# mbitsnbites/himg

Measured on NVIDIA B200. Metric: encode+decode megapixels/sec, higher is better.
Workload: dtype int16

## Files before the change

himg_b200/csrc/api.cu:

```cuda
#include <cuda_runtime.h>

#include <algorithm>
#include <chrono>
#include <cstdlib>
#include <cstdarg>
#include <cstdio>
#include <cstring>
#include <map>
#include <mutex>
#include <string>
#include <thread>
#include <vector>

#include "../../include/himg_cuda.h"
#include "huff_dec_kernels.cuh"
#include "huff_enc_kernels.cuh"
#include "tables.h"
#include "xform_fwd3.cuh"
#include "xform_inv2.cuh"
#include "xform_avg2.cuh"
#include "xform_inv4.cuh"
#include "xform_kernels.cuh"

using namespace himgcu;

namespace {

__global__ void k_store_u32(uint32_t *__restrict__ dst, const uint32_t *__restrict__ src, int n) {
  const int i = blockIdx.x * blockDim.x + threadIdx.x;
  if (i < n) dst[i] = src[i];
}

struct DevBuf {
  void *p = nullptr;
  size_t cap = 0;
};

struct ProfRec {
  const char *name;
  cudaEvent_t a, b;
};

}

struct himgcu_ctx {
  int device = 0;
  cudaStream_t own_stream = nullptr;
  cudaStream_t stream = nullptr;
  cudaStream_t in_stream = nullptr, out_stream = nullptr;
  cudaStream_t aux_stream = nullptr;
  cudaEvent_t ev_fork = nullptr, ev_join = nullptr;
  static constexpr int kMaxLanes = 8;
  std::vector<himgcu_ctx *> lanes;
  int host_lanes = 3;
  cudaEvent_t ev_in[kMaxLanes] = {}, ev_cmp[kMaxLanes] = {}, ev_out[kMaxLanes] = {};
  std::string err;
  std::map<std::string, DevBuf> bufs;
  DevBuf full_lut;
  DevBuf signed_lut;
  void *pinned = nullptr;
  size_t pinned_cap = 0;
  void *stage[2] = {nullptr, nullptr};
  cudaEvent_t stage_ev[2] = {nullptr, nullptr};
  bool profile = false;
  std::vector<ProfRec> pending;
  std::vector<cudaEvent_t> event_pool;
  std::map<std::string, std::pair<double, int>> prof;
  std::vector<std::string> prof_names;
  uint64_t launches = 0;
  size_t max_workspace = (size_t)24 << 30;
  int item_lists = 1;
  size_t host_sub_bytes = (size_t)192 << 20;
  bool force_generic = false;
  int xform_variant = 0;
  std::string lowres_key, prefix_key;
};

namespace {

int fail(himgcu_ctx *c, int code, const char *fmt, ...) {
  char buf[512];
  va_list ap;
  va_start(ap, fmt);
  vsnprintf(buf, sizeof(buf), fmt, ap);
  va_end(ap);
  if (c) c->err = buf;
  return code;
}

#define CK(call)                                                                              \
  do {                                                                                        \
    cudaError_t e_ = (call);                                                                  \
    if (e_ != cudaSuccess)                                                                    \
      return fail(ctx, HIMGCU_ERR_CUDA, "%s failed: %s (%s:%d)", #call, cudaGetErrorString(e_), \
                  __FILE__, __LINE__);                                                        \
  } while (0)

int ensure(himgcu_ctx *ctx, const char *name, size_t bytes, void **out) {
  DevBuf &b = ctx->bufs[name];
  if (b.cap < bytes) {
    if (b.p) {
      CK(cudaStreamSynchronize(ctx->stream));
      CK(cudaFree(b.p));
      b.p = nullptr;
      b.cap = 0;
    }
    const size_t want = (bytes + 255) & ~(size_t)255;
    CK(cudaMalloc(&b.p, want));
    b.cap = want;
    ctx->lowres_key.clear();
    ctx->prefix_key.clear();
  }
  *out = b.p;
  return HIMGCU_OK;
}

#define ENSURE(name, bytes, ptr)                                             \
  do {                                                                       \
    void *p_ = nullptr;                                                      \
    int rc_ = ensure(ctx, name, (bytes), &p_);                               \
    if (rc_ != HIMGCU_OK) return rc_;                                        \
    ptr = reinterpret_cast<decltype(ptr)>(p_);                               \
  } while (0)

cudaEvent_t get_event(himgcu_ctx *ctx) {
  if (!ctx->event_pool.empty()) {
    cudaEvent_t e = ctx->event_pool.back();
    ctx->event_pool.pop_back();
    return e;
  }
  cudaEvent_t e;
  cudaEventCreate(&e);
  return e;
}

struct LaunchScope {
  himgcu_ctx *ctx;
  const char *name;
  cudaEvent_t a = nullptr, b = nullptr;
  LaunchScope(himgcu_ctx *c, const char *n) : ctx(c), name(n) {
    ++ctx->launches;
    if (ctx->profile) {
      a = get_event(ctx);
      b = get_event(ctx);
      cudaEventRecord(a, ctx->stream);
    }
  }
  ~LaunchScope() {
    if (ctx->profile) {
      cudaEventRecord(b, ctx->stream);
      ctx->pending.push_back({name, a, b});
    }
  }
};
// ... 335 lines not shown
  const int total_pairs = g.rows * (g.cols / 2);
  constexpr int TP = NCH == 1 ? kInv4ThreadsGray : kInv4ThreadsRgb;
  dim3 grid((total_pairs + TP - 1) / TP, 1, n);
  const int smem = NCH * 64 * 2 * TP + kInvTableBytes;
  CK(cudaFuncSetAttribute((k_inverse4<NCH, TP>), cudaFuncAttributeMaxDynamicSharedMemorySize, smem));
  const uint32_t pr_magic = (uint32_t)((1ull << 32) / (unsigned)(g.cols / 2)) + 1u;
  LAUNCH("k_inverse", (k_inverse4<NCH, TP>), grid, TP, smem, d_planes, d_R, g, d_inv, inv_stride, d_pixels, 1u, pr_magic);
  return HIMGCU_OK;
}

int stage_inverse(himgcu_ctx *ctx, const uint8_t *d_planes, const uint8_t *d_R, int n, const Geom &g,
                  const DecTables *d_tabs, unsigned long long tab_stride, uint8_t *d_pixels) {
  if (!ctx->force_generic && !(ctx->xform_variant & 1) && (g.h % 8) == 0 && (g.cols % 16) == 0 && (g.w % 16) == 0 &&
      (g.nch == 1 || g.nch == 3) && (reinterpret_cast<uintptr_t>(d_planes) & 15) == 0 &&
      (reinterpret_cast<uintptr_t>(d_pixels) & 15) == 0 && (reinterpret_cast<uintptr_t>(d_R) & 1) == 0) {
    if (g.nch == 1) return launch_inv4<1>(ctx, d_planes, d_R, n, g, d_tabs, tab_stride, d_pixels);
    return launch_inv4<3>(ctx, d_planes, d_R, n, g, d_tabs, tab_stride, d_pixels);
  }
  if (!ctx->force_generic && (g.w % 8) == 0 && (g.h % 8) == 0 && (g.cols % 16) == 0 &&
      (reinterpret_cast<uintptr_t>(d_planes) & 15) == 0 && (reinterpret_cast<uintptr_t>(d_pixels) & 7) == 0 &&
      (((size_t)g.w * g.nch) & 7) == 0) {
    switch (g.nch) {
      case 1: return launch_inv2<1>(ctx, d_planes, d_R, n, g, d_tabs, tab_stride, d_pixels);
      case 3: return launch_inv2<3>(ctx, d_planes, d_R, n, g, d_tabs, tab_stride, d_pixels);
      case 4: return launch_inv2<4>(ctx, d_planes, d_R, n, g, d_tabs, tab_stride, d_pixels);
      default: break;
    }
  }
  switch (g.nch) {
    case 1: return launch_inv<1>(ctx, d_planes, d_R, n, g, d_tabs, tab_stride, d_pixels);
    case 2: return launch_inv<2>(ctx, d_planes, d_R, n, g, d_tabs, tab_stride, d_pixels);
    case 3: return launch_inv<3>(ctx, d_planes, d_R, n, g, d_tabs, tab_stride, d_pixels);
    case 4: return launch_inv<4>(ctx, d_planes, d_R, n, g, d_tabs, tab_stride, d_pixels);
    default: break;
  }
  int rc = launch_inv<3>(ctx, d_planes, d_R, n, g, d_tabs, tab_stride, d_pixels, 0, g.nch);
  for (int c = 3; c < g.nch && !rc; ++c) rc = launch_inv<1>(ctx, d_planes, d_R, n, g, d_tabs, tab_stride, d_pixels, c, g.nch);
  return rc;
}

struct HuffChunkArgs {
  const uint8_t *d_in;
  HuffGeom hg;
  const char *tag;
  std::vector<uint8_t> prefix;
  int size_patch;
};

int huff_encode_items(himgcu_ctx *ctx, int n, HuffChunkArgs *chunks, int nchunks, bool riff, uint8_t *d_out,
                      size_t out_stride, uint32_t *d_sizes) {
  int *d_err;
  const bool fresh = ctx->bufs.find("enc_err") == ctx->bufs.end() || ctx->bufs["enc_err"].p == nullptr;
  ENSURE("enc_err", sizeof(int), d_err);
  if (fresh) CK(cudaMemsetAsync(d_err, 0, sizeof(int), ctx->stream));
  LayoutParams P;
  memset(&P, 0, sizeof(P));
  P.nchunks = nchunks;
  P.riff_patch = riff ? 1 : 0;
  P.out = d_out;
  P.out_stride = out_stride;
  P.sizes = d_sizes;
  P.err = d_err;
  size_t prefix_total = 0;
  for (int k = 0; k < nchunks; ++k) prefix_total += chunks[k].prefix.size();
  uint8_t *d_prefix = nullptr;
  if (prefix_total) {
    ENSURE("enc_prefix", prefix_total, d_prefix);
    std::vector<uint8_t> all;
    for (int k = 0; k < nchunks; ++k) all.insert(all.end(), chunks[k].prefix.begin(), chunks[k].prefix.end());
    const std::string key(all.begin(), all.end());
    if (ctx->prefix_key != key) {
      CK(cudaMemcpyAsync(d_prefix, all.data(), all.size(), cudaMemcpyHostToDevice, ctx->stream));
      CK(cudaStreamSynchronize(ctx->stream));
      ctx->prefix_key = key;
    }
  }
  size_t prefix_off = 0;
  TreeOut *d_trees[2];
  uint32_t *d_seghist[2], *d_bits[2], *d_pos[2];
  uint32_t *d_part[2], *d_pbits[2];
  TreeParams TP;
  memset(&TP, 0, sizeof(TP));
  ItemLists lists[2];
  for (int k = 0; k < nchunks; ++k) {
    HuffGeom &hg = chunks[k].hg;
    hg.nsub = 1;
    hg.sub_size = hg.seg_size;
    const long long ctas = (long long)n * hg.nseg, fill = hg.nseg == 1 ? 148 * 8 : 148 * 2;
    if (!ctx->force_generic && ctas < fill && hg.seg_size > 2 * kTokPiece) {
      const int want = (int)std::min<long long>(64, (fill + ctas - 1) / ctas);
      const int sub = (int)((((long long)hg.seg_size + want - 1) / want + kTokPiece - 1) / kTokPiece) * kTokPiece;
      hg.sub_size = sub;
      hg.nsub = (hg.seg_size + sub - 1) / sub;
    }
    const std::string tag = chunks[k].tag;
    ENSURE((tag + "_seghist").c_str(), (size_t)n * hg.nseg * hg.nsub * kSyms * sizeof(uint32_t), d_seghist[k]);
    ENSURE((tag + "_partstart").c_str(), (size_t)n * hg.nseg * hg.nsub * sizeof(uint32_t), d_part[k]);
    ENSURE((tag + "_trees").c_str(), (size_t)n * sizeof(TreeOut), d_trees[k]);
    ENSURE((tag + "_segbits").c_str(), (size_t)n * hg.nseg * sizeof(uint32_t), d_bits[k]);
    ENSURE((tag + "_segpos").c_str(), (size_t)n * hg.nseg * sizeof(uint32_t), d_pos[k]);
    dim3 grid(hg.nseg * hg.nsub, n);
    ItemLists &il = lists[k];
    il = ItemLists{nullptr, nullptr, nullptr, 0};
    if (!ctx->force_generic && ctx->item_lists) {
      const int ppp = (hg.sub_size + kTokPiece - 1) / kTokPiece;
      const size_t slots = (size_t)n * hg.nseg * hg.nsub * ppp;
      ENSURE((tag + "_itpos").c_str(), slots * kItemCap * sizeof(unsigned short), il.pos);
      ENSURE((tag + "_itval").c_str(), slots * kItemCap, il.val);
      ENSURE((tag + "_itcnt").c_str(), slots * sizeof(uint32_t), il.count);
      il.pieces_per_part = ppp;
    }
    ENSURE((tag + "_partbits").c_str(), (size_t)n * hg.nseg * hg.nsub * sizeof(uint32_t), d_pbits[k]);
    uint32_t *d_total = nullptr;
    if (!ctx->force_generic) {
      ENSURE((tag + "_histtotal").c_str(), (size_t)n * kSyms * sizeof(uint32_t), d_total);
      CK(cudaMemsetAsync(d_total, 0, (size_t)n * kSyms * sizeof(uint32_t), ctx->stream));
    }
    if (ctx->force_generic) LAUNCH("k_huff_hist", k_huff_hist, grid, kHuffThreads, 0, chunks[k].d_in, hg, d_seghist[k]);
    else LAUNCH("k_huff_hist", k_huff_hist2, grid, kTokThreads, 0, chunks[k].d_in, hg, d_seghist[k], il, d_total);
    TP.total[k] = d_total;
    TP.seghist[k] = d_seghist[k];
    TP.trees[k] = d_trees[k];
    TP.rows[k] = hg.nseg * hg.nsub;
    LayoutChunk &C = P.ch[k];
    C.part_bits = d_pbits[k];
    C.seghist = d_seghist[k];
    C.trees = d_trees[k];
    C.seg_bits = d_bits[k];
    C.seg_pos = d_pos[k];
    C.part_start = d_part[k];
    C.nsub = hg.nsub;
    C.prefix = chunks[k].prefix.empty() ? nullptr : d_prefix + prefix_off;
    C.prefix_len = (int)chunks[k].prefix.size();
    C.size_patch = chunks[k].size_patch;
    C.nseg = hg.nseg;
    C.framed = hg.nseg > 1 ? 1 : 0;
    prefix_off += chunks[k].prefix.size();
  }
  LAUNCH("k_huff_tree", k_huff_tree, dim3(n, nchunks), kTreeThreads, 0, TP, d_err);
  for (int k = 0; k < nchunks; ++k) {
    const int rows = chunks[k].hg.nseg * chunks[k].hg.nsub;
    LAUNCH("k_huff_layout", k_huff_segbits, dim3((rows + 7) / 8, n), 256, 0, d_seghist[k], d_trees[k], rows, d_pbits[k]);
  }
  LAUNCH("k_huff_layout", k_huff_layout, n, kLayoutThreads, 0, P);
  const size_t win_bytes = (kWinWords + 2) * sizeof(uint32_t);
  if (ctx->force_generic)
    CK(cudaFuncSetAttribute(k_huff_pack, cudaFuncAttributeMaxDynamicSharedMemorySize, (int)win_bytes));
  for (int k = 0; k < nchunks; ++k) {
    const HuffGeom &hg = chunks[k].hg;
    dim3 grid(hg.nseg * hg.nsub, n);
    if (ctx->force_generic)
      LAUNCH("k_huff_pack", k_huff_pack, grid, kHuffThreads, win_bytes, chunks[k].d_in, hg, d_trees[k], d_bits[k],
             d_pos[k], d_sizes, d_out, (unsigned long long)out_stride, d_err);
    else
      LAUNCH("k_huff_pack", k_huff_pack3, grid, kTokThreads, 0, chunks[k].d_in, hg, d_trees[k], d_bits[k], d_pos[k],
             d_part[k], d_sizes, d_out, (unsigned long long)out_stride, d_err, lists[k]);
    if (hg.nseg > 1) {
      LAUNCH("k_huff_stale", k_huff_stale, dim3((hg.nseg + 255) / 256, n), 256, 0, n, hg.nseg, d_bits[k], d_pos[k], d_sizes,
             d_out, (unsigned long long)out_stride);
    }
  }
  return HIMGCU_OK;
}

int read_err_flag(himgcu_ctx *ctx, const char *name, int *value) {
  int *d_err;
  ENSURE(name, sizeof(int), d_err);
  CK(cudaMemcpyAsync(value, d_err, sizeof(int), cudaMemcpyDeviceToHost, ctx->stream));
  CK(cudaMemsetAsync(d_err, 0, sizeof(int), ctx->stream));
  CK(cudaStreamSynchronize(ctx->stream));
  return HIMGCU_OK;
}

int enc_err_status(himgcu_ctx *ctx, int err) {
  if (err == 5) return fail(ctx, HIMGCU_ERR_UNSUPPORTED, "Huffman code longer than 32 bits");
  if (err == 99) return fail(ctx, HIMGCU_ERR_CUDA, "internal: packed size mismatch");
  if (err) return fail(ctx, HIMGCU_ERR_CAPACITY, "internal output bound exceeded");
  return HIMGCU_OK;
}

size_t per_image_encode_ws(const Geom &g) {
  return 2 * (size_t)g.nch * g.rows * g.cols + g.lres_stride + g.planes_bytes +
         (size_t)(g.rows + 1) * kSyms * 4 + 2 * sizeof(TreeOut) + (size_t)(g.rows + 1) * 8 +
         ((size_t)g.rows * ((g.seg + kTokPiece - 1) / kTokPiece) + (g.lres_size + kTokPiece - 1) / kTokPiece + 64) *
             (kItemCap * 3 + 4);
}

int encode_device(himgcu_ctx *ctx, const uint8_t *d_pixels, int n, const Geom &g, int quality, bool ycbcr,
                  uint8_t *d_out, size_t out_stride, uint32_t *d_sizes) {
  EncodeTables t;
  BuildEncodeTables(quality, ycbcr, &t);
  ContainerTemplate ct;
  BuildContainerTemplate(t, g.w, g.h, g.nch, &ct);
  uint8_t *d_L, *d_lres, *d_planes;
  ENSURE("L", (size_t)n * g.nch * g.rows * g.cols, d_L);
  ENSURE("lres", (size_t)n * g.lres_stride, d_lres);
  ENSURE("planes", (size_t)n * g.planes_bytes, d_planes);
  int rc = stage_lowres(ctx, d_pixels, n, g, ycbcr, d_L);
  if (rc) return rc;
  rc = stage_lres_encode(ctx, d_L, n, g, t, d_lres);
  if (rc) return rc;
  rc = stage_forward(ctx, d_pixels, d_L, n, g, t, d_planes);
  if (rc) return rc;
  HuffChunkArgs ch[2];
  ch[0].d_in = d_lres;
  ch[0].hg = HuffGeom{g.lres_size, g.lres_size, 1, g.lres_stride, 1, g.lres_size};
  ch[0].tag = "lres";
  ch[0].prefix = ct.head;
  ch[0].size_patch = (int)ct.head.size() - 4;
  ch[1].d_in = d_planes;
  ch[1].hg = HuffGeom{(int)g.planes_bytes, g.seg, g.rows, g.planes_bytes, 1, g.seg};
  ch[1].tag = "fres";
  ch[1].prefix = ct.mid;
  ch[1].size_patch = (int)ct.mid.size() - 4;
  return huff_encode_items(ctx, n, ch, 2, true, d_out, out_stride, d_sizes);
}

int decode_team(long long streams, int out_bytes, int base) {
  int team = base;
  while (team < kParMaxTeam && streams * team < 131072 && out_bytes / (team * 2) >= 256) team *= 2;
  return team;
}

constexpr int kDecCluster = 8;
bool use_decode_cluster(long long streams, int out_bytes) { return streams <= 16 && out_bytes >= (64 << 10); }
int launch_stream_cluster(himgcu_ctx *ctx, const char *name, int n, const uint8_t *d_in, const ChunkDesc *d_cd,
                          const DecTree *d_tree, const SegRef *d_seg, int out_seg, uint8_t *d_out,
                          unsigned long long out_stride, int *d_status, bool *launched) {
  const int threads = out_seg >= (256 << 10) ? 512 : 256;
  cudaLaunchConfig_t cfg = {};
  cfg.gridDim = dim3(kDecCluster, n);
  cfg.blockDim = dim3(threads);
  cfg.stream = ctx->stream;
  cudaLaunchAttribute at[1];
  at[0].id = cudaLaunchAttributeClusterDimension;
  at[0].val.clusterDim.x = kDecCluster;
// ... 128 lines not shown
    CK(cudaEventCreateWithFlags(&ctx->ev_in[b], cudaEventDisableTiming));
    CK(cudaEventCreateWithFlags(&ctx->ev_cmp[b], cudaEventDisableTiming));
    CK(cudaEventCreateWithFlags(&ctx->ev_out[b], cudaEventDisableTiming));
  }
  return HIMGCU_OK;
}

int ensure_pinned(himgcu_ctx *ctx, size_t bytes) {
  if (ctx->pinned_cap >= bytes) return HIMGCU_OK;
  if (ctx->pinned) {
    CK(cudaStreamSynchronize(ctx->stream));
    CK(cudaFreeHost(ctx->pinned));
    ctx->pinned = nullptr;
    ctx->pinned_cap = 0;
  }
  CK(cudaMallocHost(&ctx->pinned, bytes));
  ctx->pinned_cap = bytes;
  return HIMGCU_OK;
}

struct PipeTrace {
  bool on = getenv("HIMG_DEBUG_PIPE") != nullptr;
  const char *tag;
  std::vector<cudaEvent_t> ev;
  std::vector<double> host;
  static double now() {
    return std::chrono::duration<double, std::milli>(std::chrono::steady_clock::now().time_since_epoch()).count();
  }
  static double &host_epoch() {
    static double t = 0;
    return t;
  }
  static cudaEvent_t epoch() {
    static cudaEvent_t e = [] {
      cudaEvent_t x;
      cudaEventCreate(&x);
      cudaEventRecord(x, 0);
      cudaEventSynchronize(x);
      host_epoch() = now();
      return x;
    }();
    return e;
  }
  void launched(int k) {
    if (!on) return;
    if ((int)host.size() <= k) host.resize(k + 1, 0);
    host[k] = now() - host_epoch();
  }
  explicit PipeTrace(const char *t) : tag(t) {
    if (on) epoch();
  }
  void mark(int k, int what, cudaStream_t s) {
    if (!on) return;
    if ((int)ev.size() < 4 * (k + 1)) ev.resize(4 * (k + 1), nullptr);
    cudaEventCreate(&ev[4 * k + what]);
    cudaEventRecord(ev[4 * k + what], s);
  }
  ~PipeTrace() {
    if (!on) return;
    for (size_t k = 0; k * 4 < ev.size(); ++k) {
      float t[4] = {-1, -1, -1, -1};
      for (int j = 0; j < 4; ++j)
        if (ev[4 * k + j]) {
          cudaEventSynchronize(ev[4 * k + j]);
          cudaEventElapsedTime(&t[j], epoch(), ev[4 * k + j]);
          cudaEventDestroy(ev[4 * k + j]);
        }
      fprintf(stderr, "[pipe %s] sub %2zu  in %8.2f..%8.2f  coded %8.2f  out %8.2f  (launched by the host at %8.2f)\n", tag, k,
              t[0], t[1], t[2], t[3], k < host.size() ? host[k] : -1.0);
    }
  }
};

int prepare_lanes(himgcu_ctx *ctx, int K, int *count) {
  int S = std::max(1, std::min({ctx->host_lanes, (int)himgcu_ctx::kMaxLanes, K}));
  if (ctx->profile) S = 1;
  while ((int)ctx->lanes.size() < S - 1) {
    himgcu_ctx *l = nullptr;
    if (himgcu_create(ctx->device, &l) != HIMGCU_OK) return fail(ctx, HIMGCU_ERR_CUDA, "cannot create a coding lane");
    ctx->lanes.push_back(l);
  }
  for (himgcu_ctx *l : ctx->lanes) {
    l->force_generic = ctx->force_generic;
    l->max_workspace = ctx->max_workspace;
  }
  *count = S;
  return HIMGCU_OK;
}
himgcu_ctx *lane_of(himgcu_ctx *ctx, int b) { return b == 0 ? ctx : ctx->lanes[b - 1]; }

int finish_lanes(himgcu_ctx *ctx, int S) {
  for (int b = 0; b < S; ++b) CK(cudaStreamSynchronize(lane_of(ctx, b)->stream));
  for (himgcu_ctx *l : ctx->lanes) {
    ctx->launches += l->launches;
    l->launches = 0;
  }
  return HIMGCU_OK;
}

template <class FIn, class FRun, class FOut>
int run_pipeline_steps(himgcu_ctx *ctx, int K, int S, cudaStream_t q_in, cudaStream_t q_out, FIn copy_in, FRun run, FOut copy_out) {
  int n_in = 0, n_run = 0, n_out = 0;
  auto done = [&](cudaEvent_t e, bool *ok) -> int {
    const cudaError_t q = cudaEventQuery(e);
    if (q != cudaSuccess && q != cudaErrorNotReady) CK(q);
    *ok = q == cudaSuccess;
    return HIMGCU_OK;
  };
  while (n_out < K) {
    bool progressed = false, ok = false;
    int rc;
    if (n_out < n_run) {
      const int b = n_out % S;
      if ((rc = done(ctx->ev_cmp[b], &ok))) return rc;
      if (ok) {
        if ((rc = copy_out(n_out, b))) return rc;
        CK(cudaEventRecord(ctx->ev_out[b], q_out));
        ++n_out;
        progressed = true;
      }
    }
    if (n_run < n_in) {
      const int b = n_run % S;
      if ((rc = done(ctx->ev_in[b], &ok))) return rc;
      if (ok && n_run >= S && (rc = done(ctx->ev_out[b], &ok))) return rc;
      if (ok) {
        himgcu_ctx *L = lane_of(ctx, b);
        if ((rc = run(n_run, b, L))) {
          if (L != ctx) ctx->err = L->err;
          return rc;
        }
        CK(cudaEventRecord(ctx->ev_cmp[b], L->stream));
        ++n_run;
        progressed = true;
      }
    }
    if (n_in < K && n_in < n_out + S && n_in < n_run + 2) {
      const int b = n_in % S;
      if ((rc = copy_in(n_in, b))) return rc;
      CK(cudaEventRecord(ctx->ev_in[b], q_in));
      ++n_in;
      progressed = true;
    }
    if (!progressed) std::this_thread::sleep_for(std::chrono::microseconds(20));
  }
  if (K > 0) CK(cudaEventSynchronize(ctx->ev_out[(K - 1) % S]));
  return finish_lanes(ctx, S);
}

template <class FIn, class FRun, class FOut>
int run_pipeline(himgcu_ctx *ctx, int K, int S, cudaStream_t q_in, cudaStream_t q_out, FIn copy_in, FRun run, FOut copy_out) {
  const int rc = run_pipeline_steps(ctx, K, S, q_in, q_out, copy_in, run, copy_out);
  if (rc != HIMGCU_OK) {
    const std::string why = ctx->err;
    for (int b = 0; b < S; ++b) cudaStreamSynchronize(lane_of(ctx, b)->stream);
    cudaStreamSynchronize(q_in);
    cudaStreamSynchronize(q_out);
    finish_lanes(ctx, S);
    cudaGetLastError();
    ctx->err = why;
  }
  return rc;
}

}

// ... 568 lines not shown
           d_in, d_cd, d_tree, d_seg, nseg, seg, d_out, (unsigned long long)out_stride, d_status);
  } else {
    LAUNCH("k_dec_stream", k_dec_stream_par<false>, dim3(nseg, n), team, 0, d_in, d_cd, d_tree, d_seg, nseg, seg, d_out,
           (unsigned long long)out_stride, d_status);
  }
  return HIMGCU_OK;
}

int himgcu_stage_lres_decode(himgcu_ctx *ctx, const uint8_t *d_lres, size_t lres_stride, int n, int w, int h, int nch,
                             const int16_t *unmap, uint8_t *d_R) {
  if (!ctx || !d_lres || !unmap || !d_R || n < 1 || !shape_ok(w, h, nch)) return fail(ctx, HIMGCU_ERR_ARG, "bad argument");
  CK(cudaSetDevice(ctx->device));
  Geom g = make_geom(w, h, nch, nch);
  g.lres_stride = lres_stride;
  LowResTables *d_tabs;
  int rc = upload_lowres_tables(ctx, nullptr, unmap, &d_tabs);
  if (rc) return rc;
  const long long nmb = (long long)n * g.nch * g.mrows * g.mcols;
  const unsigned blocks = (unsigned)((nmb + kLresWarps * 2 - 1) / (kLresWarps * 2));
  LAUNCH("k_lres_dpcm_dec", (k_lres_dpcm<false>), blocks, kLresWarps * 32, 0, (const uint8_t *)nullptr,
         const_cast<uint8_t *>(d_lres), d_R, g, n, (const uint8_t *)nullptr, d_tabs->unmap, (unsigned long long)0);
  return HIMGCU_OK;
}

int himgcu_stage_inverse(himgcu_ctx *ctx, const uint8_t *d_planes, const uint8_t *d_R, int n, int w, int h, int nch,
                         int use_ycbcr, const uint8_t *shift_luma, const uint8_t *shift_chroma, const int16_t *unmap,
                         uint8_t *d_pixels) {
  if (!ctx || !d_planes || !d_R || !shift_luma || !shift_chroma || !unmap || !d_pixels || n < 1 || !shape_ok(w, h, nch))
    return fail(ctx, HIMGCU_ERR_ARG, "bad argument");
  CK(cudaSetDevice(ctx->device));
  DecTables t;
  memset(&t, 0, sizeof(t));
  memcpy(t.full_unmap, unmap, sizeof(t.full_unmap));
  memcpy(t.shift[0], shift_luma, 64);
  memcpy(t.shift[1], shift_chroma, 64);
  t.ycbcr = (use_ycbcr && nch >= 3) ? 1 : 0;
  DecTables *d_t;
  ENSURE("stage_dectabs", sizeof(DecTables), d_t);
  CK(cudaMemcpyAsync(d_t, &t, sizeof(t), cudaMemcpyHostToDevice, ctx->stream));
  CK(cudaStreamSynchronize(ctx->stream));
  return stage_inverse(ctx, d_planes, d_R, n, make_geom(w, h, nch, nch), d_t, 0, d_pixels);
}


int himgcu_profile_enable(himgcu_ctx *ctx, int on) {
  if (!ctx) return HIMGCU_ERR_ARG;
  ctx->profile = on != 0;
  return HIMGCU_OK;
}

int himgcu_profile_reset(himgcu_ctx *ctx) {
  if (!ctx) return HIMGCU_ERR_ARG;
  cudaStreamSynchronize(ctx->stream);
  resolve_profile(ctx);
  ctx->prof.clear();
  ctx->prof_names.clear();
  return HIMGCU_OK;
}

int himgcu_profile_count(himgcu_ctx *ctx) {
  if (!ctx) return 0;
  cudaStreamSynchronize(ctx->stream);
  resolve_profile(ctx);
  return (int)ctx->prof_names.size();
}

int himgcu_profile_get(himgcu_ctx *ctx, int index, const char **name, double *total_ms, int *launches) {
  if (!ctx || index < 0 || index >= (int)ctx->prof_names.size()) return HIMGCU_ERR_ARG;
  const std::string &k = ctx->prof_names[index];
  if (name) *name = k.c_str();
  if (total_ms) *total_ms = ctx->prof[k].first;
  if (launches) *launches = ctx->prof[k].second;
  return HIMGCU_OK;
}

uint64_t himgcu_launch_count(himgcu_ctx *ctx) { return ctx ? ctx->launches : 0; }

int himgcu_set_option(himgcu_ctx *ctx, const char *name, long long value) {
  if (!ctx || !name) return HIMGCU_ERR_ARG;
  if (!strcmp(name, "force_generic")) ctx->force_generic = value != 0;
  else if (!strcmp(name, "xform_variant")) ctx->xform_variant = (int)value;
  else if (!strcmp(name, "max_workspace_bytes")) ctx->max_workspace = (size_t)value;
  else if (!strcmp(name, "item_lists")) ctx->item_lists = value != 0;
  else if (!strcmp(name, "host_sub_batch_bytes")) ctx->host_sub_bytes = (size_t)std::max<long long>(value, 1 << 20);
  else if (!strcmp(name, "host_lanes")) ctx->host_lanes = (int)std::max<long long>(1, std::min<long long>(value, himgcu_ctx::kMaxLanes));
  else return fail(ctx, HIMGCU_ERR_ARG, "unknown option %s", name);
  return HIMGCU_OK;
}

}
```

himg_b200/csrc/huff_enc_kernels.cuh:

```cuda
#ifndef HIMG_B200_HUFF_ENC_KERNELS_CUH_
#define HIMG_B200_HUFF_ENC_KERNELS_CUH_

#include "common.cuh"

namespace himgcu {

constexpr int kHuffThreads = 512;
constexpr int kChunkBytes = 32;
constexpr int kPieceBytes = kHuffThreads * kChunkBytes;
constexpr int kWinWords = 8192;
constexpr int kWinBits = kWinWords * 32;

struct HuffGeom {
  int in_size;
  int seg_size;
  int nseg;
  unsigned long long in_stride;
  int nsub;
  int sub_size;
};

struct TreeOut {
  uint32_t code[kSyms];
  uint32_t hist[kSyms];
// ... 896 lines not shown
            }
            wide |= l > 32;
            tok[j] = tk;
            tl[j] = l;
            tbits += l;
          }
        }
      }
      uint32_t total;
      const uint32_t tb = block_exscan_u32(tbits, ws, &total);
      if (wfill + total > (uint32_t)kWin2Bits) flush();
      const bool split = wfill + total > (uint32_t)kWin2Bits;
      if (split) {
        if (t == kTokThreads / 2) s_half = tb;
        __syncthreads();
      }
      const uint32_t half0 = split ? s_half : total;
      for (int hlf = 0; hlf < (split ? 2 : 1); ++hlf) {
        if (hlf == 1) flush();
        const bool mine = !split || (t >= kTokThreads / 2) == (hlf == 1);
        const uint32_t rel = hlf == 1 ? tb - half0 : tb;
        if (mine && m > 0) {
          uint32_t pos = wfill + rel;
          if (!wide) {
            uint32_t word = pos >> 5, fill = pos & 31;
            uint64_t acc = 0;
#pragma unroll
            for (int j = 0; j < kP3Items; ++j) {
              acc |= tok[j] << fill;
              fill += tl[j];
              if (fill >= 32) {
                atomicOr(&win[word], (uint32_t)acc);
                acc >>= 32;
                fill -= 32;
                ++word;
              }
            }
            if ((uint32_t)acc) atomicOr(&win[word], (uint32_t)acc);
          } else {
#pragma unroll
            for (int j = 0; j < kP3Items; ++j) {
              if (j < m) {
                if (tl[j] <= 64) {
                  put64(win, pos, tok[j], tl[j]);
                } else {
                  const uint2 lr = s_tab[byte_of(k0 + j, (int)ipos[k0 + j])];
                  const uint32_t rb = tl[j] - (lr.y & 255u);
                  put64(win, pos, tok[j], rb);
                  put64(win, pos + rb, lr.x, lr.y & 255u);
                }
                pos += tl[j];
              }
            }
          }
        }
        wfill += hlf == 1 ? total - half0 : half0;
      }
    }
    __syncthreads();
  }
  if (carry && part == hg.nsub - 1) {
    emit_full_runs(carry / kMaxRun);
    const uint32_t rest = carry % kMaxRun;
    if (rest) {
      uint64_t rt;
      uint32_t rb;
      run_token(s_tab, rest, &rt, &rb);
      if (wfill + rb > (uint32_t)kWin2Bits) flush();
      if (t == 0) put64(win, wfill, rt, rb);
      wfill += rb;
    }
  }
  flush();
  if (t == 0) {
    const uint32_t gbits = (first_bit & ~7u) + gbyte * 8u + wfill;
    if (wfill) {
      if (part + 1 < hg.nsub || first_shared) atomic_or_byte(dst + gbyte, win[0]);
      else dst[gbyte] = (uint8_t)win[0];
    }
    if (gbits != end_bit) atomicMax(err, 99);
  }
}

constexpr int kStaleWindow = 1024;
__global__ void __launch_bounds__(256)
    k_huff_stale(int n, int nseg, const uint32_t *__restrict__ seg_bits, const uint32_t *__restrict__ seg_pos,
                 const uint32_t *__restrict__ sizes, uint8_t *__restrict__ out, unsigned long long out_stride) {
  __shared__ uint32_t sb[kStaleWindow + 256];
  const int item = blockIdx.y, b0 = blockIdx.x * 256, b = b0 + (int)threadIdx.x;
  if (sizes[item] == 0) return;
  const uint32_t *bits = seg_bits + (size_t)item * nseg;
  const uint32_t *pos = seg_pos + (size_t)item * nseg;
  const int w0 = max(0, b0 - kStaleWindow), w1 = min(nseg, b0 + 256);
  for (int i = threadIdx.x; i < w1 - w0; i += 256) sb[i] = bits[w0 + i];
  __syncthreads();
  if (b == 0 || b >= nseg) return;
  uint32_t lo = sb[b - w0];
  const uint32_t hi = (lo + 7) & ~7u;
  if (lo == hi) return;
  uint8_t *base = out + (size_t)item * out_stride;
  const uint32_t byte_idx = lo >> 3;
  uint32_t add = 0;
  for (int e = b - 1; e >= 0 && lo < hi; --e) {
    const uint32_t le = e >= w0 ? sb[e - w0] : bits[e];
    if (le > lo) {
      const uint32_t upto = min(le, hi);
      const uint32_t mask = ((1u << (upto - (byte_idx << 3))) - 1u) & ~((1u << (lo - (byte_idx << 3))) - 1u);
      add |= base[pos[e] + byte_idx] & mask;
      lo = upto;
    }
  }
  if (add) base[pos[b] + byte_idx] |= (uint8_t)add;
}

}

#endif
```

Baseline: 72270.

## Add warp-per-segment Huffman histogram and pack kernels for many-segment inputs

Adds k_huff_hist4 and k_huff_pack4, which give each warp its own Huffman segment (8 segments per CTA) instead of one CTA per segment. A warp-level walk compacts nonzero items into a shared queue. Packing encodes 8 items per lane with a prefix sum into a small per-warp shared-memory window. The new path is chosen by default when there are multiple segments, no sub-splitting, and enough segments to fill a wave. It is meant to cut idle threads and synchronisation on sparse segments, at the cost of more frequent flushes from the smaller window and new code paths.

```diff
diff --git a/himg_b200/csrc/api.cu b/himg_b200/csrc/api.cu
--- a/himg_b200/csrc/api.cu
+++ b/himg_b200/csrc/api.cu
@@ -70,6 +70,7 @@
   uint64_t launches = 0;
   size_t max_workspace = (size_t)24 << 30;
   int item_lists = 1;
+  int huff_warp_teams = 1;
   size_t host_sub_bytes = (size_t)192 << 20;
   bool force_generic = false;
   int xform_variant = 0;
@@ -571,6 +572,7 @@
   TreeParams TP;
   memset(&TP, 0, sizeof(TP));
   ItemLists lists[2];
+  bool teams[2] = {false, false};
   for (int k = 0; k < nchunks; ++k) {
     HuffGeom &hg = chunks[k].hg;
     hg.nsub = 1;
@@ -582,6 +584,9 @@
       hg.sub_size = sub;
       hg.nsub = (hg.seg_size + sub - 1) / sub;
     }
+    const long long wave = 148LL * kTeamWarps * kP4MinCtas;
+    teams[k] = !ctx->force_generic && hg.nseg > 1 && hg.nsub == 1 &&
+               (ctx->huff_warp_teams == 2 || (ctx->huff_warp_teams == 1 && (long long)n * hg.nseg >= wave));
     const std::string tag = chunks[k].tag;
     ENSURE((tag + "_seghist").c_str(), (size_t)n * hg.nseg * hg.nsub * kSyms * sizeof(uint32_t), d_seghist[k]);
     ENSURE((tag + "_partstart").c_str(), (size_t)n * hg.nseg * hg.nsub * sizeof(uint32_t), d_part[k]);
@@ -606,6 +611,9 @@
       CK(cudaMemsetAsync(d_total, 0, (size_t)n * kSyms * sizeof(uint32_t), ctx->stream));
     }
     if (ctx->force_generic) LAUNCH("k_huff_hist", k_huff_hist, grid, kHuffThreads, 0, chunks[k].d_in, hg, d_seghist[k]);
+    else if (teams[k])
+      LAUNCH("k_huff_hist", k_huff_hist4, dim3((hg.nseg + kTeamWarps - 1) / kTeamWarps, n), kTeamThreads, 0, chunks[k].d_in,
+             hg, d_seghist[k], il, d_total);
     else LAUNCH("k_huff_hist", k_huff_hist2, grid, kTokThreads, 0, chunks[k].d_in, hg, d_seghist[k], il, d_total);
     TP.total[k] = d_total;
     TP.seghist[k] = d_seghist[k];
@@ -635,12 +643,16 @@
   const size_t win_bytes = (kWinWords + 2) * sizeof(uint32_t);
   if (ctx->force_generic)
     CK(cudaFuncSetAttribute(k_huff_pack, cudaFuncAttributeMaxDynamicSharedMemorySize, (int)win_bytes));
+  if (teams[0] || teams[1]) CK(cudaFuncSetAttribute(k_huff_pack4, cudaFuncAttributeMaxDynamicSharedMemorySize, kP4Smem));
   for (int k = 0; k < nchunks; ++k) {
     const HuffGeom &hg = chunks[k].hg;
     dim3 grid(hg.nseg * hg.nsub, n);
     if (ctx->force_generic)
       LAUNCH("k_huff_pack", k_huff_pack, grid, kHuffThreads, win_bytes, chunks[k].d_in, hg, d_trees[k], d_bits[k],
              d_pos[k], d_sizes, d_out, (unsigned long long)out_stride, d_err);
+    else if (teams[k])
+      LAUNCH("k_huff_pack", k_huff_pack4, dim3((hg.nseg + kTeamWarps - 1) / kTeamWarps, n), kTeamThreads, kP4Smem, chunks[k].d_in,
+             hg, d_trees[k], d_bits[k], d_pos[k], d_sizes, d_out, (unsigned long long)out_stride, d_err, lists[k]);
     else
       LAUNCH("k_huff_pack", k_huff_pack3, grid, kTokThreads, 0, chunks[k].d_in, hg, d_trees[k], d_bits[k], d_pos[k],
              d_part[k], d_sizes, d_out, (unsigned long long)out_stride, d_err, lists[k]);
@@ -935,6 +947,8 @@
   }
   for (himgcu_ctx *l : ctx->lanes) {
     l->force_generic = ctx->force_generic;
+    l->item_lists = ctx->item_lists;
+    l->huff_warp_teams = ctx->huff_warp_teams;
     l->max_workspace = ctx->max_workspace;
   }
   *count = S;
@@ -1669,6 +1683,7 @@
   else if (!strcmp(name, "xform_variant")) ctx->xform_variant = (int)value;
   else if (!strcmp(name, "max_workspace_bytes")) ctx->max_workspace = (size_t)value;
   else if (!strcmp(name, "item_lists")) ctx->item_lists = value != 0;
+  else if (!strcmp(name, "huff_warp_teams")) ctx->huff_warp_teams = (int)std::max<long long>(0, std::min<long long>(value, 2));
   else if (!strcmp(name, "host_sub_batch_bytes")) ctx->host_sub_bytes = (size_t)std::max<long long>(value, 1 << 20);
   else if (!strcmp(name, "host_lanes")) ctx->host_lanes = (int)std::max<long long>(1, std::min<long long>(value, himgcu_ctx::kMaxLanes));
   else return fail(ctx, HIMGCU_ERR_ARG, "unknown option %s", name);
diff --git a/himg_b200/csrc/huff_enc_kernels.cuh b/himg_b200/csrc/huff_enc_kernels.cuh
--- a/himg_b200/csrc/huff_enc_kernels.cuh
+++ b/himg_b200/csrc/huff_enc_kernels.cuh
@@ -1002,6 +1002,359 @@
   }
 }
 
+constexpr int kTeamWarps = 8;
+constexpr int kTeamThreads = kTeamWarps * 32;
+constexpr int kWalkStep = 32 * 16;
+
+__device__ __forceinline__ uint4 load16(const uint8_t *__restrict__ seg, int seg_size, int off, bool aligned) {
+  if (aligned && off + 16 <= seg_size) return __ldg(reinterpret_cast<const uint4 *>(seg + off));
+  uint32_t w[4] = {0, 0, 0, 0};
+#pragma unroll
+  for (int k = 0; k < 16; ++k)
+    if (off + k < seg_size) w[k >> 2] |= (uint32_t)seg[off + k] << (8 * (k & 3));
+  return make_uint4(w[0], w[1], w[2], w[3]);
+}
+
+template <int kRound, class Consume>
+__device__ __forceinline__ int warp_walk_items(const uint8_t *__restrict__ seg, int seg_size, int *qpos, uint8_t *qval,
+                                               Consume &&consume) {
+  const int lane = threadIdx.x & 31;
+  const bool aligned = (reinterpret_cast<uintptr_t>(seg) & 15) == 0;
+  if (lane == 0) qpos[0] = -1;
+  __syncwarp();
+  int qn = 0, g0 = 0;
+  uint4 nxt = load16(seg, seg_size, 16 * lane, aligned);
+  for (int base = 0; base < seg_size; base += kWalkStep) {
+    const int off = base + 16 * lane;
+    const uint4 w = nxt;
+    nxt = load16(seg, seg_size, off + kWalkStep, aligned);
+    uint32_t m = nonzero_nibble(w.x) | nonzero_nibble(w.y) << 4 | nonzero_nibble(w.z) << 8 | nonzero_nibble(w.w) << 12;
+    const uint32_t c = __popc(m);
+    uint32_t inc = c;
+#pragma unroll
+    for (int d = 1; d < 32; d <<= 1) {
+      const uint32_t t = __shfl_up_sync(0xffffffffu, inc, d);
+      if (lane >= d) inc += t;
+    }
+    const int step_items = (int)__shfl_sync(0xffffffffu, inc, 31);
+    if (step_items == 0) continue;
+    int k = 1 + qn + (int)(inc - c);
+    while (m) {
+      const int j = __ffs(m) - 1;
+      m &= m - 1;
+      const uint32_t word = j < 4 ? w.x : (j < 8 ? w.y : (j < 12 ? w.z : w.w));
+      qpos[k] = off + j;
+      qval[k] = (uint8_t)(word >> (8 * (j & 3)));
+      ++k;
+    }
+    qn += step_items;
+    __syncwarp();
+    if (qn >= kRound) {
+      int done = 0;
+      for (; qn - done >= kRound; done += kRound) consume(done, kRound, g0 + done);
+      __syncwarp();
+      for (int i = lane; i <= qn - done; i += 32) {
+        qpos[i] = qpos[done + i];
+        qval[i] = qval[done + i];
+      }
+      g0 += done;
+      qn -= done;
+      __syncwarp();
+    }
+  }
+  if (qn) consume(0, qn, g0);
+  return qpos[qn];
+}
+
+__device__ __forceinline__ size_t seg_list_base(const ItemLists &L, int nseg, int item, int b) {
+  return ((size_t)item * nseg + b) * ((size_t)L.pieces_per_part * kItemCap);
+}
+
+__global__ void __launch_bounds__(kTeamThreads)
+    k_huff_hist4(const uint8_t *__restrict__ in, HuffGeom hg, uint32_t *__restrict__ seghist, ItemLists lists,
+                 uint32_t *__restrict__ total) {
+  constexpr int kQ = 32 + kWalkStep;
+  __shared__ uint32_t sh[kTeamWarps][kSyms];
+  __shared__ int qpos_all[kTeamWarps][kQ];
+  __shared__ uint8_t qval_all[kTeamWarps][kQ];
+  const int wid = threadIdx.x >> 5, lane = threadIdx.x & 31, item = blockIdx.y;
+  const int b = blockIdx.x * kTeamWarps + wid;
+  if (b >= hg.nseg) return;
+  uint32_t *h = sh[wid];
+  int *qpos = qpos_all[wid];
+  uint8_t *qval = qval_all[wid];
+  for (int i = lane; i < kSyms; i += 32) h[i] = 0;
+  __syncwarp();
+  const uint8_t *seg = in + (size_t)item * hg.in_stride + (size_t)b * hg.seg_size;
+  const bool lists_on = lists.pieces_per_part != 0;
+  const int cap = lists.pieces_per_part * kItemCap;
+  unsigned short *lpos = lists_on ? lists.pos + seg_list_base(lists, hg.nseg, item, b) : nullptr;
+  uint8_t *lval = lists_on ? lists.val + seg_list_base(lists, hg.nseg, item, b) : nullptr;
+  bool long_gap = false;
+  auto run = [&](uint32_t z) {
+    if (z >= (uint32_t)kMaxRun) {
+      atomicAdd(&h[260], z / kMaxRun);
+      z %= kMaxRun;
+    }
+    uint32_t ex;
+    if (z) atomicAdd(&h[run_symbol(z, &ex)], 1u);
+  };
+  int nitems = 0;
+  const int last = warp_walk_items<32>(seg, hg.seg_size, qpos, qval, [&](int k0, int cnt, int g0) {
+    nitems = g0 + cnt;
+    if (lane < cnt) {
+      const int k = k0 + lane;
+      const uint32_t gap = (uint32_t)(qpos[1 + k] - qpos[k] - 1), v = qval[1 + k];
+      run(gap);
+      atomicAdd(&h[v], 1u);
+      long_gap |= gap > 0xffffu;
+      if (lists_on && g0 + lane < cap) {
+        lpos[g0 + lane] = (unsigned short)gap;
+        lval[g0 + lane] = (uint8_t)v;
+      }
+    }
+  });
+  if (lane == 0) run((uint32_t)(hg.seg_size - 1 - last));
+  __syncwarp();
+  if (lists_on) {
+    const bool stored = nitems <= cap && !__any_sync(0xffffffffu, long_gap);
+    if (lane == 0) lists.count[(size_t)item * hg.nseg + b] = stored ? (uint32_t)nitems : kItemsNotStored;
+  }
+  uint32_t *dst = seghist + ((size_t)item * hg.nseg + b) * kSyms;
+  for (int i = lane; i < kSyms; i += 32) {
+    const uint32_t v = h[i];
+    dst[i] = v;
+    if (total && v) atomicAdd(&total[(size_t)item * kSyms + i], v);
+  }
+}
+
+constexpr int kP4Items = 8;
+constexpr int kP4Round = 32 * kP4Items;
+constexpr int kWin4Words = 512;
+constexpr int kWin4Bits = kWin4Words * 32;
+constexpr int kP4Queue = kP4Round + kWalkStep;
+constexpr int kP4MinCtas = 4;
+constexpr int kP4Smem = kTeamWarps * ((kWin4Words + 4) * 4 + kP4Queue * 5);
+
+__global__ void __launch_bounds__(kTeamThreads, kP4MinCtas)
+    k_huff_pack4(const uint8_t *__restrict__ in, HuffGeom hg, const TreeOut *__restrict__ trees,
+                 const uint32_t *__restrict__ seg_bits, const uint32_t *__restrict__ seg_pos,
+                 const uint32_t *__restrict__ sizes, uint8_t *__restrict__ out, unsigned long long out_stride, int *err,
+                 ItemLists lists) {
+  extern __shared__ uint32_t p4_smem[];
+  __shared__ uint2 s_tab[kSyms];
+  const int wid = threadIdx.x >> 5, lane = threadIdx.x & 31, item = blockIdx.y;
+  if (sizes[item] == 0) return;
+  const TreeOut *tr = trees + item;
+  for (int s = threadIdx.x; s < kSyms; s += blockDim.x) {
+    const uint32_t l = tr->len[s];
+    s_tab[s] = make_uint2(tr->code[s], l | ((l + (uint32_t)sym_extra_bits(s)) << 8));
+  }
+  __syncthreads();
+  const int b = blockIdx.x * kTeamWarps + wid;
+  if (b >= hg.nseg) return;
+  uint32_t *win = p4_smem + wid * (kWin4Words + 4);
+  int *qpos = reinterpret_cast<int *>(p4_smem + kTeamWarps * (kWin4Words + 4)) + wid * kP4Queue;
+  uint8_t *qval = reinterpret_cast<uint8_t *>(p4_smem + kTeamWarps * (kWin4Words + 4 + kP4Queue)) + wid * kP4Queue;
+  for (int i = lane; i < kWin4Words + 4; i += 32) win[i] = 0;
+  __syncwarp();
+  const uint8_t *seg = in + (size_t)item * hg.in_stride + (size_t)b * hg.seg_size;
+  uint8_t *dst = out + (size_t)item * out_stride + seg_pos[(size_t)item * hg.nseg + b];
+  const uint32_t full_bits = s_tab[260].y >> 8;
+  const uint64_t full_tok = (uint64_t)s_tab[260].x | ((uint64_t)(kMaxRun - 279) << (s_tab[260].y & 255u));
+
+  uint32_t gbyte = 0;
+  uint32_t wfill = 0;
+  auto flush = [&]() {
+    __syncwarp();
+    const uint32_t nbytes = wfill >> 3;
+    const uint8_t *wb = reinterpret_cast<const uint8_t *>(win);
+    for (uint32_t i = lane; i < nbytes; i += 32) dst[gbyte + i] = wb[i];
+    const uint32_t keep = (wfill & 7) ? wb[nbytes] : 0u;
+    __syncwarp();
+    const uint32_t used = min((wfill >> 5) + 4u, (uint32_t)(kWin4Words + 4));
+    for (uint32_t i = lane; i < used; i += 32) win[i] = i == 0 ? keep : 0u;
+    __syncwarp();
+    gbyte += nbytes;
+    wfill &= 7;
+  };
+  auto put_uniform = [&](uint64_t v, uint32_t n) {
+    if (wfill + n > (uint32_t)kWin4Bits) flush();
+    if (lane == 0) put64(win, wfill, v, n);
+    wfill += n;
+  };
+  auto run_uniform = [&](uint32_t z) {
+    for (uint32_t nfull = z / kMaxRun; nfull;) {
+      const uint32_t cap = ((uint32_t)kWin4Bits - wfill) / full_bits;
+      if (cap == 0) {
+        flush();
+        continue;
+      }
+      const uint32_t n = min(nfull, cap);
+      if (lane == 0)
+        for (uint32_t i = 0; i < n; ++i) put64(win, wfill + i * full_bits, full_tok, full_bits);
+      wfill += n * full_bits;
+      nfull -= n;
+    }
+    const uint32_t rest = z % kMaxRun;
+    if (rest) {
+      uint64_t rt;
+      uint32_t rb;
+      run_token(s_tab, rest, &rt, &rb);
+      put_uniform(rt, rb);
+    }
+  };
+  auto round = [&](int m, auto &&fetch8, auto &&fetch1) {
+    uint64_t tok[kP4Items];
+    uint32_t tl[kP4Items];
+    uint32_t tbits = 0;
+    bool wide = false;
+    uint32_t gap[kP4Items], val[kP4Items];
+    fetch8(gap, val);
+#pragma unroll
+    for (int j = 0; j < kP4Items; ++j) {
+      tok[j] = 0;
+      tl[j] = 0;
+      if (j < m) {
+        const uint2 lr = s_tab[val[j]];
+        uint64_t tk = lr.x;
+        uint32_t l = lr.y & 255u;
+        const uint32_t nfull = gap[j] / kMaxRun, z = gap[j] - nfull * kMaxRun;
+        if (z) {
+          uint64_t rt;
+          uint32_t rb;
+          run_token(s_tab, z, &rt, &rb);
+          tk = rt | (tk << rb);
+          l += rb;
+        }
+        wide |= l > 32 || nfull;
+        l += nfull * full_bits;
+        tok[j] = tk;
+        tl[j] = l;
+        tbits += l;
+      }
+    }
+    uint32_t inc = tbits;
+#pragma unroll
+    for (int d = 1; d < 32; d <<= 1) {
+      const uint32_t t = __shfl_up_sync(0xffffffffu, inc, d);
+      if (lane >= d) inc += t;
+    }
+    const uint32_t total = __shfl_sync(0xffffffffu, inc, 31);
+    if (wfill + total > (uint32_t)kWin4Bits) flush();
+    if (wfill + total > (uint32_t)kWin4Bits) {
+      for (int L = 0; L < 32; ++L) {
+        const int mL = __shfl_sync(0xffffffffu, m, L);
+#pragma unroll
+        for (int j = 0; j < mL; ++j) {
+          uint32_t g, v;
+          fetch1(kP4Items * L + j, g, v);
+          run_uniform(g);
+          put_uniform(s_tab[v].x, s_tab[v].y & 255u);
+        }
+      }
+      return;
+    }
+    uint32_t pos = wfill + inc - tbits;
+    if (!wide) {
+      uint32_t word = pos >> 5, fill = pos & 31;
+      uint64_t acc = 0;
+#pragma unroll
+      for (int j = 0; j < kP4Items; ++j) {
+        acc |= tok[j] << fill;
+        fill += tl[j];
+        if (fill >= 32) {
+          atomicOr(&win[word], (uint32_t)acc);
+          acc >>= 32;
+          fill -= 32;
+          ++word;
+        }
+      }
+      if ((uint32_t)acc) atomicOr(&win[word], (uint32_t)acc);
+    } else {
+#pragma unroll
+      for (int j = 0; j < kP4Items; ++j) {
+        if (j < m) {
+          uint32_t g, v;
+          fetch1(kP4Items * lane + j, g, v);
+          const uint32_t nfull = g / kMaxRun, z = g - nfull * kMaxRun;
+          for (uint32_t f = 0; f < nfull; ++f, pos += full_bits) put64(win, pos, full_tok, full_bits);
+          if (z) {
+            uint64_t rt;
+            uint32_t rb;
+            run_token(s_tab, z, &rt, &rb);
+            put64(win, pos, rt, rb);
+            pos += rb;
+          }
+          const uint2 lr = s_tab[v];
+          put64(win, pos, lr.x, lr.y & 255u);
+          pos += lr.y & 255u;
+        }
+      }
+    }
+    wfill += total;
+  };
+
+  int last;
+  const uint32_t cnt = lists.pieces_per_part ? lists.count[(size_t)item * hg.nseg + b] : kItemsNotStored;
+  if (cnt != kItemsNotStored) {
+    const size_t lb = seg_list_base(lists, hg.nseg, item, b);
+    const uint4 *gp = reinterpret_cast<const uint4 *>(lists.pos + lb);
+    const uint2 *gv = reinterpret_cast<const uint2 *>(lists.val + lb);
+    uint32_t span = 0;
+    uint4 np = make_uint4(0, 0, 0, 0);
+    uint2 nv = make_uint2(0, 0);
+    if (kP4Items * lane < (int)cnt) np = __ldg(gp + lane), nv = __ldg(gv + lane);
+    for (int r0 = 0; r0 < (int)cnt; r0 += kP4Round) {
+      const int k0 = r0 + kP4Items * lane, m = min(max((int)cnt - k0, 0), kP4Items);
+      const uint4 p = np;
+      const uint2 v = nv;
+      if (k0 + kP4Round < (int)cnt) np = __ldg(gp + (k0 + kP4Round) / kP4Items), nv = __ldg(gv + (k0 + kP4Round) / kP4Items);
+      round(
+          m,
+          [&](uint32_t(&gap)[kP4Items], uint32_t(&val)[kP4Items]) {
+            const uint32_t pw[4] = {p.x, p.y, p.z, p.w}, vw[2] = {v.x, v.y};
+#pragma unroll
+            for (int j = 0; j < kP4Items; ++j) {
+              gap[j] = (pw[j >> 1] >> (16 * (j & 1))) & 0xffffu;
+              val[j] = (vw[j >> 2] >> (8 * (j & 3))) & 0xffu;
+              if (j < m) span += gap[j] + 1;
+            }
+          },
+          [&](int k, uint32_t &g, uint32_t &val) {
+            g = lists.pos[lb + r0 + k];
+            val = lists.val[lb + r0 + k];
+          });
+    }
+    last = (int)__reduce_add_sync(0xffffffffu, span) - 1;
+  } else {
+    last = warp_walk_items<kP4Round>(seg, hg.seg_size, qpos, qval, [&](int k0, int n, int) {
+      const int m = min(max(n - kP4Items * lane, 0), kP4Items);
+      auto fetch1 = [&](int k, uint32_t &g, uint32_t &val) {
+        g = (uint32_t)(qpos[1 + k0 + k] - qpos[k0 + k] - 1);
+        val = qval[1 + k0 + k];
+      };
+      round(
+          m,
+          [&](uint32_t(&gap)[kP4Items], uint32_t(&val)[kP4Items]) {
+#pragma unroll
+            for (int j = 0; j < kP4Items; ++j) {
+              gap[j] = 0;
+              val[j] = 0;
+              if (j < m) fetch1(kP4Items * lane + j, gap[j], val[j]);
+            }
+          },
+          fetch1);
+    });
+  }
+  run_uniform((uint32_t)(hg.seg_size - 1 - last));
+  flush();
+  if (lane == 0) {
+    if (wfill) dst[gbyte] = (uint8_t)win[0];
+    if (gbyte * 8u + wfill != seg_bits[(size_t)item * hg.nseg + b]) atomicMax(err, 99);
+  }
+}
+
 constexpr int kStaleWindow = 1024;
 __global__ void __launch_bounds__(256)
     k_huff_stale(int n, int nseg, const uint32_t *__restrict__ seg_bits, const uint32_t *__restrict__ seg_pos,
```

Measured after the change: 78920, median of 6. 9.2% higher.
